# CogSP/CoEvoNet

Hardware: AMD Instinct MI355X
Metric: env-steps/sec (agent-steps of the whole job; generations/sec in gens_per_sec), Co-GA simple_adversary_v3 pop=200 HoF=5 (higher is better)
Workload: dtype f32

## Files before the change

### coevonet_amd/csrc/coevo_common.hip.h

```cpp
#pragma once
#include <hip/hip_runtime.h>
#include <stdint.h>

#include "../../include/coevo.h"

namespace coevo {

constexpr int H1 = COEVO_FC_H1;
constexpr int H2 = COEVO_FC_H2;
constexpr int NACT = COEVO_FC_NACT;
constexpr float LN_EPS = 1e-5f;

__host__ __device__ constexpr int64_t fc_off_b1(int D) { return (int64_t)D * H1; }
__host__ __device__ constexpr int64_t fc_off_w2(int D) { return fc_off_b1(D) + 3 * H1; }
__host__ __device__ constexpr int64_t fc_off_b2(int D) { return fc_off_w2(D) + (int64_t)H1 * H2; }
__host__ __device__ constexpr int64_t fc_off_w3(int D) { return fc_off_b2(D) + 3 * H2; }
__host__ __device__ constexpr int64_t fc_off_b3(int D) { return fc_off_w3(D) + NACT * H2; }
__host__ __device__ constexpr int64_t fc_params(int D) { return fc_off_b3(D) + NACT; }
__host__ __device__ constexpr int64_t fc_stride(int D) { return (fc_params(D) + 63) / 64 * 64; }

__host__ __device__ inline int64_t fc_slab_to_flat(int64_t s, int D)
{
    const int64_t o_b1 = fc_off_b1(D), o_w2 = fc_off_w2(D), o_b2 = fc_off_b2(D);
    if (s < o_b1) {
        int64_t k = s / H1, j = s % H1;
        return j * D + k;
    }
    if (s < o_w2) return s;
    if (s < o_b2) {
        int64_t t = s - o_w2;
        int64_t c = t & 3, l = (t >> 2) & 63, kq = (t >> 8) & 127, jb = t >> 15;
        return o_w2 + (jb * 64 + l) * H1 + kq * 4 + c;
    }
    return s;
}

template <int CTRL>
__device__ inline float dpp_move(float v)
{
    return __int_as_float(__builtin_amdgcn_mov_dpp(__float_as_int(v), CTRL, 0xf, 0xf, true));
}

__device__ inline float row16_tree_sum(float v)
{
    v = v + dpp_move<0xB1>(v);
    v = v + dpp_move<0x4E>(v);
    v = v + dpp_move<0x141>(v);
    v = v + dpp_move<0x140>(v);
    return v;
// ... 272 lines not shown
```

### coevonet_amd/csrc/fc_forward.hip

```cpp
#include <cstdlib>

#include "coevo_common.hip.h"

namespace coevo {

#ifndef COEVO_HEAVY16_U
#define COEVO_HEAVY16_U 4
#endif
#ifndef COEVO_LIGHT_U
#define COEVO_LIGHT_U 8
#endif

typedef float f32x4_t __attribute__((ext_vector_type(4)));
__device__ inline float4 load_stream16(const float4 *p)
{
#ifdef COEVO_NO_NT
    return *p;
#else
    const f32x4_t v = __builtin_nontemporal_load(reinterpret_cast<const f32x4_t *>(p));
    return make_float4(v[0], v[1], v[2], v[3]);
#endif
}

template <int R, int P>
// ... 1027 lines not shown
    fc_policy_mfma_body<MODE>(a, sm, a.tasks[blockIdx.x]);
}

struct FcMfma16Smem {
    union {
        float h1a[H1][16];
        float h2[16][260];
    };
    float xst[12][16];
    float w3s[NACT][260];
    float red[16][8];
    float logit[16][COEVO_LOGIT_STRIDE];
};
static_assert(sizeof(FcMfma16Smem) <= 40960, "four workgroups per CU");

template <int MODE>
__device__ __forceinline__ void fc_policy_mfma16_body(const FcArgs &a, FcMfma16Smem &sm, const coevo_fc_task &task)
{
    typedef float f32x4_acc __attribute__((ext_vector_type(4)));
    typedef unsigned u32x2_s __attribute__((ext_vector_type(2)));
    COEVO_STAMP(0);
    const int t = threadIdx.x, w = t >> 6, l = t & 63, lc = l & 15, lg = l >> 4;
    const int D = task.D, nrows = task.n_rows, row0 = task.row_begin;
    const float *net = a.slab + task.net_off;
    int st = 0;

    constexpr int KS = 3;
    float *par = &sm.h1a[0][0];
    {
        const int n_pieces = (D + 3) * (H1 / 4);
#pragma unroll
        for (int j = 0; j < 7; ++j)
            if (64 * w + 256 * j < n_pieces)
                __builtin_amdgcn_global_load_lds((const __attribute__((address_space(1))) void *)(net + 4 * (t + 256 * j)),
                                                 (__attribute__((address_space(3))) void *)(par + 4 * (64 * w + 256 * j)),
// ... 124 lines not shown
            if (row < nrows && bad_post_relu(y)) st |= COEVO_ST_BAD_FC1;
            const int k = 128 * w + 16 * T + lc;
            sm.h1a[k][row ^ ((k >> 2) & 3)] = relu_keep_nan(y);
        }
    }
    asm volatile("" : "+v"(st));
    __syncthreads();
    COEVO_STAMP(2);

    f32x4_acc c2[4];
    {
#pragma unroll
        for (int T = 0; T < 4; ++T)
#pragma unroll
            for (int i = 0; i < 4; ++i) c2[T][i] = p_b2[T];
        const float4 *wp = reinterpret_cast<const float4 *>(net + fc_off_w2(D)) + (size_t)w * 128 * 64 + l;
        constexpr int U = COEVO_HEAVY16_U;
        float4 bufA[U], bufB[U];
        auto issue = [&](float4 (&buf)[U], int kq) {
#pragma unroll
            for (int u = 0; u < U; ++u) buf[u] = wp[(size_t)(kq + u) * 64];
        };
        auto consume = [&](const float4 (&buf)[U], int kq) {
#pragma unroll
            for (int u = 0; u < U; ++u) {
                const int q = kq + u;
                const float av = sm.h1a[4 * q + lg][lc ^ (q & 3)];
                const u32x2_s s02 = __builtin_amdgcn_permlane32_swap(__float_as_uint(buf[u].x), __float_as_uint(buf[u].z), false, false);
                const u32x2_s s13 = __builtin_amdgcn_permlane32_swap(__float_as_uint(buf[u].y), __float_as_uint(buf[u].w), false, false);
                const u32x2_s y01 = __builtin_amdgcn_permlane16_swap(s02[0], s13[0], false, false);
                const u32x2_s y23 = __builtin_amdgcn_permlane16_swap(s02[1], s13[1], false, false);
                c2[0] = __builtin_amdgcn_mfma_f32_16x16x4f32(av, __uint_as_float(y01[0]), c2[0], 0, 0, 0);
                c2[1] = __builtin_amdgcn_mfma_f32_16x16x4f32(av, __uint_as_float(y01[1]), c2[1], 0, 0, 0);
                c2[2] = __builtin_amdgcn_mfma_f32_16x16x4f32(av, __uint_as_float(y23[0]), c2[2], 0, 0, 0);
                c2[3] = __builtin_amdgcn_mfma_f32_16x16x4f32(av, __uint_as_float(y23[1]), c2[3], 0, 0, 0);
            }
        };
        issue(bufA, 0);
        int kq = 0;
        for (; kq < 128 - 2 * U; kq += 2 * U) {
            issue(bufB, kq + U);
            __builtin_amdgcn_sched_barrier(0);
            consume(bufA, kq);
            issue(bufA, kq + 2 * U);
            __builtin_amdgcn_sched_barrier(0);
            consume(bufB, kq + U);
        }
        issue(bufB, kq + U);
        __builtin_amdgcn_sched_barrier(0);
        consume(bufA, kq);
// ... 82 lines not shown
}

template <int R, int MODE = MODE_FUSED>
__global__ __launch_bounds__(256, 4) void fc_cycle16_kernel(FcArgs a)
{
    __shared__ __attribute__((aligned(16))) union Cycle16Smem {
        FcMfma16Smem heavy;
#if COEVO_COMPACT
        FcSmemC<R> light;
#else
        FcSmem<R, 1> light;
#endif
    } sm;
    static_assert(sizeof(sm) <= 40960, "four workgroups per CU");
    stamp_begin(a.stamps);
    if ((int)blockIdx.x < a.n_heavy)
        fc_policy_mfma16_body<MODE>(a, sm.heavy, a.tasks[blockIdx.x]);
    else
#if COEVO_COMPACT
    {
        const int li = (int)blockIdx.x - a.n_heavy;
        if (MODE == MODE_FUSED && li < a.n_light && (a.light_tasks[li].reserved & COEVO_TASK_RESIDENT))
            fc_policy_body_c<R, MODE, FC2_MFMA, MODE == MODE_FUSED>(a, sm.light, a.light_tasks, li, a.n_light);
        else
            fc_policy_body_c<R, MODE>(a, sm.light, a.light_tasks, li, a.n_light);
    }
#else
        fc_policy_body<R, MODE, 1>(a, sm.light, a.light_tasks, (int)blockIdx.x - a.n_heavy, a.n_light);
#endif
    stamp_end(a.stamps);
}

template <int R, int MODE = MODE_FUSED>
// ... 684 lines not shown
```

### coevonet_amd/csrc/offspring.hip

```cpp
#include "coevo_common.hip.h"
#include "dqn_common.hip.h"
#include "philox.hip.h"

namespace coevo {

__device__ inline bool fc_slab_is_layernorm(int64_t s, int D)
{
    const int64_t g1 = fc_off_b1(D) + H1, g2 = fc_off_b2(D) + H2;
    return (s >= g1 && s < g1 + 2 * H1) || (s >= g2 && s < g2 + 2 * H2);
}

__device__ inline void slab_quad_normals(uint64_t seed, uint32_t slo, uint32_t shi, int64_t s0, int D, int64_t P,
                                         float z[4])
{
    int64_t p[4];
#pragma unroll
    for (int i = 0; i < 4; ++i) p[i] = (s0 + i < P) ? fc_slab_to_flat(s0 + i, D) : -1;
    float zz[4];
    int64_t have = -1;
#pragma unroll
    for (int i = 0; i < 4; ++i) {
        if (p[i] < 0) { z[i] = 0.0f; continue; }
        const int64_t q = p[i] >> 2;
        if (q != have) { philox_normal4(seed, slo, shi, (uint32_t)q, zz); have = q; }
// ... 130 lines not shown
    *reinterpret_cast<float4 *>(dst_slab + (int64_t)(dst_first + c) * stride + s0) = v;
}

struct GaPromoteArgs {
    coevo_ga_promote_role role[3];
    int E, hof;
    const float *sigma;
    const int32_t *gen_dev;
    uint64_t seed;
    uint32_t stream_hi_prev;
    int32_t *tick;
};
constexpr int PROMOTE_MAX_E = 8, PROMOTE_MAX_HOF = 16;

template <int I>
__device__ __forceinline__ void promote_hof_shift(float *hof, int64_t stride, int64_t s0, int n)
{
    if constexpr (I < PROMOTE_MAX_HOF) {
        const float4 v = *reinterpret_cast<const float4 *>(hof + (int64_t)(I < n ? I : n - 1) * stride + s0);
        promote_hof_shift<I + 1>(hof, stride, s0, n);
        *reinterpret_cast<float4 *>(hof + (int64_t)(I < n ? I - 1 : n - 1) * stride + s0) = v;
    }
}

template <int K>
__device__ __forceinline__ float4 promote_elites(const float *src, const int32_t *order, float *elite, bool store,
                                                 int64_t stride, int64_t s0, int E)
{
    if constexpr (K < PROMOTE_MAX_E) {
        const int kc = K < E ? K : E - 1;
        const float4 v = *reinterpret_cast<const float4 *>(src + (int64_t)(order ? order[kc] : kc) * stride + s0);
        promote_elites<K + 1>(src, order, elite, store, stride, s0, E);
        if (store) *reinterpret_cast<float4 *>(elite + (int64_t)kc * stride + s0) = v;
        return v;
    } else {
        return make_float4(0.f, 0.f, 0.f, 0.f);
// ... 23 lines not shown
        }
        *reinterpret_cast<float4 *>(elite + (int64_t)kc * stride + s0) = nv;
        return nv;
    } else {
        return make_float4(0.f, 0.f, 0.f, 0.f);
    }
}

__global__ __launch_bounds__(256) void ga_promote_kernel(GaPromoteArgs a)
{
    const unsigned y = blockIdx.y;
#define PROMOTE_SEL(f) (y == 0 ? a.role[0].f : (y == 1 ? a.role[1].f : a.role[2].f))
    float *pop = PROMOTE_SEL(pop), *hof = PROMOTE_SEL(hof), *elite = PROMOTE_SEL(elite);
    const int32_t *order = PROMOTE_SEL(order);
    const int D = PROMOTE_SEL(D), from_pop = PROMOTE_SEL(elites_from_pop), to_pop0 = PROMOTE_SEL(best_to_pop0);
#undef PROMOTE_SEL
    const int64_t stride = fc_stride(D);
    const int64_t s0 = ((int64_t)blockIdx.x * 256 + threadIdx.x) * 4;
    if (s0 >= stride) return;
    float4 e0;
    if (a.sigma && !from_pop) {
        uint32_t shi = a.stream_hi_prev + y;
        if (a.gen_dev) shi += 4u * (uint32_t)(*a.gen_dev - 1);
        e0 = promote_rebuild<0>(elite, order, stride, s0, a.E, D, a.sigma[y], a.seed, shi);
    } else {
        e0 = from_pop ? promote_elites<0>(pop, order, elite, true, stride, s0, a.E)
                      : *reinterpret_cast<const float4 *>(elite + s0);
    }
    promote_hof_shift<1>(hof, stride, s0, a.hof);
    *reinterpret_cast<float4 *>(hof + (int64_t)(a.hof - 1) * stride + s0) = e0;
    if (to_pop0) *reinterpret_cast<float4 *>(pop + s0) = e0;
    if (a.tick && blockIdx.x == 0 && blockIdx.y == 0 && threadIdx.x == 0) *a.tick += 1;
}

__global__ __launch_bounds__(256) void es_update_kernel(float *theta, const float *pert_slab, int D,
                                                         const float *fitness, int n, const float *sigma_dev, float lr)
{
    const int64_t stride = fc_stride(D), P = fc_params(D);
    const int64_t s0 = ((int64_t)blockIdx.x * 256 + threadIdx.x) * 4;
    if (s0 >= stride) return;
    const float sigma = *sigma_dev;
    const float scale = lr / ((float)n * sigma);
    const float4 tv = *reinterpret_cast<const float4 *>(theta + s0);
    const float th[4] = {tv.x, tv.y, tv.z, tv.w};
    float acc[4] = {0.0f, 0.0f, 0.0f, 0.0f};
// ... 242 lines not shown
                               int n, int D, void *stream)
{
    if (!src_slab || !src_idx || !dst_slab || !fc_dim_ok(D) || n < 0 || dst_first < 0 || n > 65535)
        return COEVO_ERR_ARG;
    if (n == 0) return COEVO_OK;
    const dim3 grid((unsigned)((fc_stride(D) / 4 + 255) / 256), (unsigned)n);
    hipLaunchKernelGGL(fc_gather_kernel, grid, dim3(256), 0, (hipStream_t)stream, src_slab, src_idx, dst_slab,
                       dst_first, fc_stride(D));
    COEVO_HIP_CHECK(hipGetLastError());
    return COEVO_OK;
}

static int ga_promote_launch(const coevo_ga_promote_role *roles, int n_roles, int E, int hof, const float *sigma,
                             uint64_t seed, uint32_t stream_hi_prev, const int32_t *gen_dev, int32_t *tick, void *stream);

extern "C" int coevo_ga_promote(const coevo_ga_promote_role *roles, int n_roles, int E, int hof, void *stream)
{
    return ga_promote_launch(roles, n_roles, E, hof, nullptr, 0, 0, nullptr, nullptr, stream);
}

extern "C" int coevo_ga_promote_tick(const coevo_ga_promote_role *roles, int n_roles, int E, int hof, int32_t *counter,
                                     void *stream)
{
    if (!counter) return COEVO_ERR_ARG;
    return ga_promote_launch(roles, n_roles, E, hof, nullptr, 0, 0, nullptr, counter, stream);
}

extern "C" int coevo_ga_promote_rebuild(const coevo_ga_promote_role *roles, int n_roles, int E, int hof, const float *sigma,
                                        uint64_t seed, uint32_t stream_hi_prev, const int32_t *gen_dev, void *stream)
{
// ... 1 lines not shown
    for (int r = 0; roles && r < n_roles && r < 3; ++r)
        if (!roles[r].elites_from_pop && !roles[r].order) return COEVO_ERR_ARG;
    return ga_promote_launch(roles, n_roles, E, hof, sigma, seed, stream_hi_prev, gen_dev, nullptr, stream);
}

static int ga_promote_launch(const coevo_ga_promote_role *roles, int n_roles, int E, int hof, const float *sigma,
                             uint64_t seed, uint32_t stream_hi_prev, const int32_t *gen_dev, int32_t *tick, void *stream)
{
    if (!roles || n_roles < 1 || n_roles > 3 || E < 1 || E > PROMOTE_MAX_E || hof < 1 || hof > PROMOTE_MAX_HOF)
        return COEVO_ERR_ARG;
    GaPromoteArgs a{};
    a.sigma = sigma; a.seed = seed; a.stream_hi_prev = stream_hi_prev; a.gen_dev = gen_dev; a.tick = tick;
    int64_t max_stride = 0;
    for (int r = 0; r < n_roles; ++r) {
        const coevo_ga_promote_role &R = roles[r];
        if (!R.pop || !R.hof || !R.elite || !fc_dim_ok(R.D) || (R.elites_from_pop && !R.order)) return COEVO_ERR_ARG;
        a.role[r] = R;
        if (fc_stride(R.D) > max_stride) max_stride = fc_stride(R.D);
    }
    a.E = E; a.hof = hof;
    const dim3 grid((unsigned)((max_stride / 4 + 255) / 256), (unsigned)n_roles);
    hipLaunchKernelGGL(ga_promote_kernel, grid, dim3(256), 0, (hipStream_t)stream, a);
    COEVO_HIP_CHECK(hipGetLastError());
    return COEVO_OK;
}

extern "C" int coevo_es_update(float *theta_slab_net, const float *pert_slab, int D, const float *fitness, int n,
                               const float *sigma_dev, float lr, void *stream)
{
    if (!theta_slab_net || !pert_slab || !fitness || !sigma_dev || !fc_dim_ok(D) || n <= 0) return COEVO_ERR_ARG;
    const dim3 grid((unsigned)((fc_stride(D) / 4 + 255) / 256));
// ... 141 lines not shown
```

### coevonet_amd/genetic_algorithm.py

```python
from __future__ import annotations

import os
import time

import numpy as np
import torch

from . import lib as L
from .fcnetwork import FCNetwork
from .game_logic import create_agent
from .mpe.simple_adversary import ENV_SEED
from .rollout import DeviceRollout, HostEnvRollout, RolloutPlan, effective_steps

ROLES = ("agent_0", "agent_1", "adversary_0")
ROLE_D = {"agent_0": 10, "agent_1": 10, "adversary_0": 8}
ROLE_SLOT = {"agent_0": 1, "agent_1": 2, "adversary_0": 0}
RET_SLOT = {"agent_0": 0, "agent_1": 1, "adversary_0": 2}
SIGMA_ATTR = {"agent_0": "mutation_power_agent_0", "agent_1": "mutation_power_agent_1",
              "adversary_0": "mutation_power_adversary"}
N_EVAL = 10


def evaluate_current_weights(agent_0, agent_1, adversary, env, args):
    from .game_logic import play_game
# ... 47 lines not shown
    return bounds, np.searchsorted(bounds[1:], np.arange(n_local), side="right").astype(np.int32)


RESIDENT_MB_DEFAULT = 224


def resident_budget_bytes():
    v = os.environ.get("COEVO_RESIDENT_MB", "").strip().lower()
    if v == "all":
        return float("inf")
    return (float(v) if v else RESIDENT_MB_DEFAULT) * 1e6


def resident_enabled(env, heavy_rows, n_local, pop):
    return env == "device" and heavy_rows == 16 and n_local >= pop


def resident_prefix(budget_bytes, fixed_bytes, individual_bytes, bounds):
    K = len(bounds) - 1
    sizes = np.diff(np.asarray(bounds, dtype=np.int64))
    left = budget_bytes - fixed_bytes
    if left <= 0 or K <= 0:
        return np.zeros(K, dtype=np.int64)
    if left == float("inf"):
        return sizes
    return np.minimum(sizes, int(left // (K * individual_bytes)))


DEFAULT_COHORTS = 1
DEVICE_LOOP_COHORTS = 2
# ... 15 lines not shown
        if self.world > 1 and pop % self.world:
            raise ValueError(f"population {pop} is not divisible by the number of ranks {self.world}")
        self.lo = self.rank * pop // self.world
        self.hi = (self.rank + 1) * pop // self.world
        self.n_local = self.hi - self.lo
        self.T_train = effective_steps(limit_train, max_cycles)
        self.T_eval = effective_steps(limit_eval, max_cycles)
        self.n_cycles = (max(self.T_train, self.T_eval) + 2) // 3
        self.first_ordinal = first_ordinal
        self.env_seed = env_seed
        self.stride = {r: L.fc_slab_stride(ROLE_D[r]) for r in ROLES}
        self.P = {r: L.fc_param_count(ROLE_D[r]) for r in ROLES}
        self.base, off = {}, 0
        for r in ROLES:
            self.base[r] = {}
            for region, count in (("pop", pop), ("hof", hof), ("elite", elites), ("stale", 1), ("hof_tmp", hof),
                                  ("elite_prev", elites)):
                self.base[r][region] = off
                off += count * self.stride[r]
        self.slab = torch.zeros(off, dtype=torch.float32, device=device)
        net_off, net_D, ids = [], [], {}

        def net(region, role, i):
            key = (region, role, i)
            if key not in ids:
                ids[key] = len(net_off)
                net_off.append(self.base[role][region] + i * self.stride[role])
                net_D.append(ROLE_D[role])
            return ids[key]

        games = []
        h = hof
# ... 11 lines not shown
        for _ in range(N_EVAL):
            games.append((net("hof", "adversary_0", h - 1), net("hof", "agent_0", h - 1), net("hof", "agent_1", h - 1)))
        heavy_rows = int(os.environ.get("COEVO_HEAVY_ROWS", "0"))
        if heavy_rows <= 0:
            cus = torch.cuda.get_device_properties(device).multi_processor_count if (env == "device" and str(device) != "cpu") else 0
            heavy_rows = small_shard_rows(self.n_local, hof, cus, pop) if (cus and cohorts <= 1) else 16
        host_k = int(os.environ.get("COEVO_HOST_COHORTS", "0")) or max(1, min(4, len(games) // 700))
        self.K = max(1, min(int(cohorts) if env == "device" else host_k, self.n_local))
        row_order = "class" if env == "device" else "cohort"
        self._set_cohort_bounds()
        game_cohort = None
        if self.K > 1:
            per_ind = np.repeat(cohort_partition(self.n_local, self.K)[1], self.hof)
            game_cohort = np.concatenate([per_ind, per_ind, per_ind, np.full(N_EVAL, self.K - 1)]).astype(np.int32)
        resident = resident_enabled(env, heavy_rows, self.n_local, pop)

        def resident_nets():
            if not resident:
                return ()
            ind_bytes = sum(4 * self.stride[r] for r in ROLES)
            n = resident_prefix(resident_budget_bytes(), (hof + elites + 1) * ind_bytes, ind_bytes, self.cohort_bounds)
            return [ids[("pop", r, self.lo + i)] for r in ROLES for k in range(self.K)
                    for i in range(int(self.cohort_bounds[k]), int(self.cohort_bounds[k]) + int(n[k]))]

        try:
            self.plan = RolloutPlan(np.array(games), net_off, net_D, device=device, heavy_rows=heavy_rows,
                                    n_cohorts=self.K, game_cohort=game_cohort, row_order=row_order,
                                    resident_nets=resident_nets())
        except ValueError:
            self.K = 1
            self._set_cohort_bounds()
            self.plan = RolloutPlan(np.array(games), net_off, net_D, device=device, heavy_rows=heavy_rows,
                                    row_order=row_order, resident_nets=resident_nets())
        if env == "device":
            self.ro = DeviceRollout(self.plan, self.slab, env_seed=env_seed, timing_pairs=timing_pairs)
        else:
            self.ro = HostEnvRollout(self.plan, self.slab, env_seed=env_seed)
        f32 = dict(dtype=torch.float32, device=device)
        self.dist_all = torch.zeros(3, pop, **f32)
        self.dist = {r: self.dist_all[i] for i, r in enumerate(ROLES)}
        self.div = {r: torch.zeros(1, **f32) for r in ROLES}
        self.fitness = {r: torch.zeros(pop, **f32) for r in ROLES}
        self.order = {r: torch.zeros(pop, dtype=torch.int32, device=device) for r in ROLES}
        self.sigma = {r: torch.zeros(1, **f32) for r in ROLES}
        self.sigma_prev = {r: torch.zeros(1, **f32) for r in ROLES}
        self.last_reward = torch.zeros(3, pop, 3, dtype=torch.float64, device=device)
        self.pack_local = torch.zeros(3, self.n_local, 4, dtype=torch.float64, device=device)
        self.pack_all = torch.zeros(self.world, 3, self.n_local, 4, dtype=torch.float64, device=device)
        self.parent_idx = torch.tensor([c % elites for c in range(max(pop - 1, 1))], dtype=torch.int32, device=device)
        self.hof_shift_idx = torch.arange(1, max(hof, 2), dtype=torch.int32, device=device)
        self.iota = torch.arange(max(hof, elites, 2), dtype=torch.int32, device=device)
        self.generation = 0
        self.steps_per_generation = 3 * pop * hof * self.T_train + N_EVAL * self.T_eval

    def _ptr(self, role, region, i=0):
        return self.slab.data_ptr() + 4 * (self.base[role][region] + i * self.stride[role])

    def upload(self, role, region, first, flat_np):
        flat = torch.from_numpy(np.ascontiguousarray(flat_np, dtype=np.float32)).to(self.device)
        L.call("coevo_fc_pack", L._p(flat), self._ptr(role, region, first), flat.shape[0], ROLE_D[role])
        if region in ("pop", "stale"):
            self._dist_current = False
        return flat

    def download(self, role, region, first, n):
        if region == "pop":
            self.flush_breeding()
        out = torch.zeros(n, self.P[role], dtype=torch.float32, device=self.device)
        L.call("coevo_fc_unpack", self._ptr(role, region, first), L._p(out), n, ROLE_D[role])
        return out.cpu().numpy()

    def load_initial(self, pop_flat, hof_flat):
        keep = []
        for r in ROLES:
            keep.append(self.upload(r, "pop", 0, pop_flat[r]))
# ... 120 lines not shown
            L.call("coevo_fc_gather", self._ptr(r, "elite"), L._p(self.iota), self._ptr(r, "pop"), 0, 1, D)
            c_lo, c_hi = (max(self.lo, 1) - 1, self.hi - 1) if sharded else (0, self.pop - 1)
            if c_hi > c_lo:
                L.call("coevo_fc_perturb", self._ptr(r, "elite"), self.parent_idx.data_ptr() + 4 * c_lo,
                       self._ptr(r, "pop"), 1 + c_lo, c_hi - c_lo, D, L._p(self.sigma[r]), self.philox_seed, c_lo,
                       gen * 4 + ri, 0)

    def _hof_push(self, r):
        D = ROLE_D[r]
        if self.hof > 1:
            L.call("coevo_fc_gather", self._ptr(r, "hof"), L._p(self.hof_shift_idx), self._ptr(r, "hof_tmp"), 0,
                   self.hof - 1, D)
            L.call("coevo_fc_gather", self._ptr(r, "hof_tmp"), L._p(self.iota), self._ptr(r, "hof"), 0,
                   self.hof - 1, D)
        L.call("coevo_fc_gather", self._ptr(r, "elite"), L._p(self.iota), self._ptr(r, "hof"), self.hof - 1, 1, D)

    def breed_host_reference(self, env, args, sigmas):
        keep = []
        self._dist_current = False
        for r in ROLES:
            D = ROLE_D[r]
            L.call("coevo_fc_gather", self._ptr(r, "pop"), L._p(self.order[r]), self._ptr(r, "elite"), 0, self.E, D)
            self._hof_push(r)
            L.call("coevo_fc_gather", self._ptr(r, "elite"), L._p(self.iota), self._ptr(r, "pop"), 0, 1, D)
        elite_flat = {r: self.download(r, "elite", 0, self.E) for r in ROLES}
        for r in ROLES:
            children = np.empty((self.pop - 1, self.P[r]), dtype=np.float32)
            for i in range(self.pop - 1):
                child = FCNetwork(ROLE_D[r], 5, "float32")
                child.set_flat(elite_flat[r][i % self.E])
# ... 54 lines not shown
        roles = (L.GaSelectRole * 3)()
        for ri, r in enumerate(ROLES):
            roles[ri] = L.GaSelectRole(None if gathered is not None else L._p(self.dist[r]),
                                       None if gathered is not None else rewards_ptr_of(ri), L._p(self.div[r]),
                                       L._p(self.fitness[r]), L._p(self.order[r]), L._p(self.best_dist[r]),
                                       0 if gathered is not None else game_first_of(ri), RET_SLOT[r])
        ad = self._adapt_args(with_prev)
        L.call("coevo_ga_select_adapt", roles, 3, self.pop, games_per_individual, self.hof,
               L._p(gathered) if gathered is not None else None, self.n_local if gathered is not None else 0, L.C.byref(ad))

    def _promote_roles(self, elites_from_pop, best_to_pop0, tick=False):
        roles = (L.GaPromoteRole * 3)()
        for ri, r in enumerate(ROLES):
            roles[ri] = L.GaPromoteRole(self._ptr(r, "pop"), self._ptr(r, "hof"), self._ptr(r, "elite"),
                                        L._p(self.order[r]), ROLE_D[r], 1 if elites_from_pop else 0,
                                        1 if best_to_pop0 else 0, 0)
        if tick:
            L.call("coevo_ga_promote_tick", roles, 3, self.E, self.hof, L._p(self.gen_dev))
            return
        L.call("coevo_ga_promote", roles, 3, self.E, self.hof)

    def enqueue_generation(self):
        self._enqueue_resets()
        self.ro.enqueue(self.n_cycles)
        self._enqueue_selection_and_breeding()

    def _enqueue_resets(self):
        assert self.world == 1 and self.env_mode == "device"
        ro, M = self.ro, 3 * self.pop * self.hof
        per_gen, per_phase = M + N_EVAL, self.pop * self.hof
        g = L._p(self.gen_dev)
# ... 191 lines not shown
                    self._sharded_tail_post(gen, breed=breed, gen_from_device=True, packed=packed)
                graphs[key] = gr
            graphs[key].replay()
            return
        self._sharded_tail_post(gen, breed, gen_from_device=False, packed=packed)

    def _sharded_tail_post(self, gen, breed, gen_from_device, packed=False):
        ro = self.ro
        g = L._p(self.gen_dev)
        mn, mx, adaptive = self.loop_args
        if packed:
            self._select_adapt_roles(None, None, 1, gathered=self.pack_all, with_prev=True)
            pr = (L.GaPromoteRole * 3)()
            for ri, r in enumerate(ROLES):
                pr[ri] = L.GaPromoteRole(self._ptr(r, "pop"), self._ptr(r, "hof"), self._ptr(r, "elite"), L._p(self.order[r]),
                                         ROLE_D[r], 1 if gen == 0 else 0, 1 if self.lo == 0 else 0, 0)
            if gen == 0:
                L.call("coevo_ga_promote", pr, 3, self.E, self.hof)
            else:
                L.call("coevo_ga_promote_rebuild", pr, 3, self.E, self.hof, L._p(self.sigma32_prev), self.philox_seed,
                       0 if gen_from_device else (gen - 1) * 4, g if gen_from_device else None)
            if breed:
                self._breed_cohort(0, gen, gen_dev=g if gen_from_device else None, tick=True)
            else:
                L.call("coevo_counter_add", g, 1)
            return
        if self.fused_tail:
            self._select_roles(lambda ri: self.last_reward[ri].data_ptr(), lambda ri: 0, 1)
        else:
            for ph, r in enumerate(ROLES):
                L.call("coevo_sharing_score", L._p(self.dist[r]), self.pop, L._p(self.div[r]))
# ... 292 lines not shown
```

### coevonet_amd/lib.py

```python
from __future__ import annotations

import ctypes as C
import os

import numpy as np
import torch

HERE = os.path.dirname(os.path.abspath(__file__))
LIB_PATH = os.environ.get("COEVO_LIB") or os.path.join(HERE, "libcoevo.so")

OBS_STRIDE = 12
LOGIT_STRIDE = 8
FC_MAX_ROWS = 32
MPE_STATE_DOUBLES = 24
STAMP_SLOTS = 32
ST_NAMES = {1: "input contains inf or NaN", 2: "output contains inf or NaN after fc1",
            4: "output contains inf or NaN after fc2", 8: "output contains inf or NaN",
            16: "no action selected (current_best_position = -1)",
            32: "persistent rollout: a workgroup timed out waiting for the other rows of its games (COEVO_ST_SYNC_TIMEOUT)",
            64: "fp16 forward: a task with a bad width, row count or unaligned net offset was skipped (COEVO_ST_BAD_TASK)"}

DQN_LOGIT_STRIDE = 32
DQN_FC1_TILED = 0x100
DQN_MAX_ROWS = 16
DQN_TASK_DTYPE = np.dtype([("net_off", "<i8"), ("row_begin", "<i4"), ("n_rows", "<i4")])

TASK_DTYPE = np.dtype([("net_off", "<i8"), ("row_begin", "<i4"), ("n_rows", "<i4"), ("D", "<i4"),
                       ("reserved", "<i4")])
TASK_RESIDENT = 1


class PCG64State(C.Structure):
    _fields_ = [("state_hi", C.c_uint64), ("state_lo", C.c_uint64), ("inc_hi", C.c_uint64), ("inc_lo", C.c_uint64)]

    @classmethod
    def from_seed(cls, seed):
        st = np.random.PCG64(seed).state["state"]
        m = (1 << 64) - 1
        return cls(st["state"] >> 64, st["state"] & m, st["inc"] >> 64, st["inc"] & m)


class PerturbJob(C.Structure):
    _fields_ = [("parent_slab", C.c_void_p), ("parent_idx", C.c_void_p), ("child_slab", C.c_void_p),
                ("sigma_dev", C.c_void_p), ("dist_ref", C.c_void_p), ("dist_partial", C.c_void_p),
# ... 214 lines not shown
    "coevo_fc_rebuild_elites": (C.c_int, [C.c_void_p, C.c_void_p, C.c_void_p, C.c_int, C.c_int, C.c_void_p, C.c_uint64,
                                          C.c_uint32, C.c_void_p, C.c_void_p]),
    "coevo_fc_perturb_gen": (C.c_int, [C.c_void_p, C.c_void_p, C.c_void_p, C.c_int, C.c_int, C.c_int, C.c_void_p,
                                       C.c_uint64, C.c_uint32, C.c_uint32, C.c_int, C.c_void_p, C.c_void_p]),
    "coevo_fc_perturb_blocks": (C.c_int64, [C.c_int]),
    "coevo_fc_perturb_dist": (C.c_int, [C.c_void_p, C.c_void_p, C.c_void_p, C.c_int, C.c_int, C.c_int, C.c_void_p,
                                        C.c_uint64, C.c_uint32, C.c_uint32, C.c_int, C.c_void_p, C.c_void_p, C.c_void_p,
                                        C.c_void_p]),
    "coevo_fc_distance_finalize": (C.c_int, [C.c_void_p, C.c_int, C.c_int, C.c_void_p, C.c_int, C.c_void_p,
                                             C.c_void_p]),
    "coevo_gather_f32": (C.c_int, [C.c_void_p, C.c_void_p, C.c_void_p, C.c_int, C.c_void_p]),
    "coevo_ga_adapt_sigma": (C.c_int, [C.c_void_p, C.c_int, C.c_void_p, C.c_void_p, C.c_void_p, C.c_int, C.c_void_p,
                                       C.c_void_p, C.c_double, C.c_double, C.c_int, C.c_void_p]),
    "coevo_counter_add": (C.c_int, [C.c_void_p, C.c_int, C.c_void_p]),
    "coevo_fc_gather": (C.c_int, [C.c_void_p, C.c_void_p, C.c_void_p, C.c_int, C.c_int, C.c_int, C.c_void_p]),
    "coevo_es_update": (C.c_int, [C.c_void_p, C.c_void_p, C.c_int, C.c_void_p, C.c_int, C.c_void_p, C.c_float,
                                  C.c_void_p]),
    "coevo_fc_diversity": (C.c_int, [C.c_void_p, C.c_void_p, C.c_int, C.c_int, C.c_void_p, C.c_void_p, C.c_void_p]),
    "coevo_fc_distance": (C.c_int, [C.c_void_p, C.c_void_p, C.c_int, C.c_int, C.c_void_p, C.c_void_p]),
    "coevo_sharing_score": (C.c_int, [C.c_void_p, C.c_int, C.c_void_p, C.c_void_p]),
    "coevo_ga_fitness": (C.c_int, [C.c_void_p, C.c_int, C.c_int, C.c_int, C.c_int, C.c_int, C.c_void_p, C.c_void_p,
                                   C.c_void_p]),
    "coevo_rank_desc": (C.c_int, [C.c_void_p, C.c_int, C.c_void_p, C.c_void_p]),
}


def exported_symbols():
    return sorted(_SIGS)


# ... 85 lines not shown
```

### coevonet_amd/rollout.py

```python
from __future__ import annotations

import ctypes as _ct

import os

import numpy as np
import torch

from . import lib as L
from .mpe import simple_adversary as sa

LIGHT_ROWS = 8
HEAVY_ROWS = 32


class RolloutPlan:

    def __init__(self, game_nets, net_off, net_D, device="cuda", heavy_rows=HEAVY_ROWS, n_cohorts=1,
                 game_cohort=None, split_rows=None, row_order="class", resident_nets=()):
        game_nets = np.asarray(game_nets, dtype=np.int64)
        self.n_games = int(game_nets.shape[0])
        by_net = {}
        for g in range(self.n_games):
            for slot in range(3):
                by_net.setdefault(int(game_nets[g, slot]), []).append((g, slot))
        for net, rows in by_net.items():
            d = int(net_D[net])
            for g, slot in rows:
                assert d == (8 if slot == 0 else 10), "net width does not match the env slot it plays"
        if game_cohort is not None:
            cohort = np.asarray(game_cohort, dtype=np.int32)
            assert cohort.shape == (self.n_games,) and cohort.min() >= 0
            for net, rows in by_net.items():
                if len(rows) <= LIGHT_ROWS and len({int(cohort[g]) for g, _ in rows}) != 1:
# ... 15 lines not shown
                light[int(cohort[rows[0][0]])].append((net, rows))
            else:
                for k in range(self.n_cohorts):
                    mine = [(g, slot) for g, slot in rows if cohort[g] == k]
                    for i in range(0, len(mine), heavy_rows):
                        heavy[k].append((net, mine[i:i + heavy_rows]))
        heavy = [self._xcd_order(h) for h in heavy]
        self.heavy_begin_np = np.cumsum([0] + [len(h) for h in heavy]).astype(np.int32)
        self.light_begin_np = np.cumsum([0] + [len(x) for x in light]).astype(np.int32)
        assert row_order in ("class", "cohort")
        row_game, row_slot = [], []
        tasks = {"heavy": [[] for _ in range(self.n_cohorts)], "light": [[] for _ in range(self.n_cohorts)]}
        cohort_rows = np.zeros(self.n_cohorts + 1, dtype=np.int64)

        resident_nets = frozenset(int(n) for n in resident_nets)

        def number(name, k):
            for net, rows in (heavy if name == "heavy" else light)[k]:
                flags = L.TASK_RESIDENT if (name == "light" and net in resident_nets) else 0
                tasks[name][k].append((int(net_off[net]), len(row_game), len(rows), int(net_D[net]), flags))
                for g, slot in rows:
                    row_game.append(g)
                    row_slot.append(slot)

        if row_order == "class":
            for name in ("heavy", "light"):
                for k in range(self.n_cohorts):
                    number(name, k)
            self.cohort_row_begin_np = None
        else:
            for k in range(self.n_cohorts):
                number("heavy", k)
                number("light", k)
                cohort_rows[k + 1] = len(row_game)
# ... 462 lines not shown
```

### include/coevo.h

```cpp
#ifndef COEVO_H
#define COEVO_H

#include <stddef.h>
#include <stdint.h>

#ifdef __cplusplus
extern "C" {
#endif

#define COEVO_VERSION 103

#define COEVO_OK 0
#define COEVO_ERR_ARG (-1)
#define COEVO_ERR_HIP (-2)
#define COEVO_ERR_UNSUPPORTED (-3)

#define COEVO_ST_BAD_INPUT 1
#define COEVO_ST_BAD_FC1 2
#define COEVO_ST_BAD_FC2 4
#define COEVO_ST_BAD_OUT 8
#define COEVO_ST_NO_ACTION 16
#define COEVO_ST_SYNC_TIMEOUT 32
#define COEVO_ST_BAD_TASK 64

// ... 13 lines not shown
const char *coevo_build_flags(void);

int64_t coevo_fc_param_count(int D);
int64_t coevo_fc_slab_stride(int D);
int coevo_fc_pack(const float *flat, float *slab, int n, int D, void *stream);
int coevo_fc_unpack(const float *slab, float *flat, int n, int D, void *stream);

typedef struct {
    int64_t net_off;
    int32_t row_begin;
    int32_t n_rows;
    int32_t D;
    int32_t reserved;
} coevo_fc_task;
#define COEVO_TASK_RESIDENT 1

int coevo_fc_forward_argmax(const float *slab, const coevo_fc_task *tasks, int n_tasks, int max_rows_per_task,
                            const float *obs, int32_t *actions, float *logits, int32_t *status, void *stream);
int coevo_fc_forward_merged(const float *slab, const coevo_fc_task *heavy_tasks, int n_heavy, int heavy_max_rows,
                            const coevo_fc_task *light_tasks, int n_light, int light_max_rows, const float *obs,
                            int32_t *actions, float *logits, int32_t *status, void *stream);

int64_t coevo_fc16_slab_stride(int D);
int coevo_fc16_pack(const float *flat, void *slab, int n, int D, void *stream);
int coevo_fc16_unpack(const void *slab, float *flat, int n, int D, void *stream);
int coevo_fc16_forward_argmax(const void *slab, const coevo_fc_task *tasks, int n_tasks, int max_rows_per_task,
                              const float *obs, int32_t *actions, float *logits, int32_t *status, void *stream);

#define COEVO_MPE_STATE_DOUBLES 24
typedef struct {
// ... 200 lines not shown
int coevo_ga_select(const coevo_ga_select_role *roles, int n_roles, int pop, int games_per_individual, int hof,
                    void *stream);
int coevo_ga_select_gathered(const coevo_ga_select_role *roles, int n_roles, int pop, int hof, const double *gathered,
                             int n_local, void *stream);
typedef struct coevo_ga_adapt_args {
    const double *rewards; const int32_t *gen_dev; double *hist; double *sig_hist; double *sigma64; float *sigma32;
    float *sigma32_prev; double sig_min, sig_max; int32_t eval_first_game, cap, adaptive, reserved;
} coevo_ga_adapt_args;
int coevo_ga_select_adapt(const coevo_ga_select_role *roles, int n_roles, int pop, int games_per_individual, int hof,
                          const double *gathered, int n_local, const coevo_ga_adapt_args *adapt, void *stream);
typedef struct coevo_ga_promote_role {
    float *pop, *hof, *elite;
    const int32_t *order;
    int32_t D, elites_from_pop, best_to_pop0, reserved;
} coevo_ga_promote_role;
int coevo_ga_promote(const coevo_ga_promote_role *roles, int n_roles, int E, int hof, void *stream);
int coevo_ga_promote_tick(const coevo_ga_promote_role *roles, int n_roles, int E, int hof, int32_t *counter, void *stream);
int coevo_ga_promote_rebuild(const coevo_ga_promote_role *roles, int n_roles, int E, int hof, const float *sigma,
                             uint64_t seed, uint32_t stream_hi_prev, const int32_t *gen_dev, void *stream);
int coevo_fc_gather(const float *src_slab, const int32_t *src_idx, float *dst_slab, int dst_first, int n, int D,
                    void *stream);

int coevo_es_update(float *theta_slab_net, const float *pert_slab, int D, const float *fitness, int n,
                    const float *sigma_dev, float lr, void *stream);

int coevo_es_partial(const float *theta_net, const float *pert_slab_local, int ind_first, int D,
                     const float *fitness_all, int n_total, int chunks_total, int chunk_first, int n_chunks,
                     float *partial, void *stream);
int coevo_es_apply(float *theta_net, const float *partials, int chunks_total, int chunks_per_block,
                   int64_t block_stride_floats, int D, int n_total, const float *sigma_dev, float lr, void *stream);
// ... 103 lines not shown
```

Baseline: 147.8 million.

## Keep pre-swizzled W2 twin copies of hall-of-fame nets to skip lane permutes

Adds a twin region holding the W2 weights of each hall-of-fame network already permuted into MFMA operand order. The copy is kept up to date on upload, on rebuild and during promote shifts. Heavy forward tasks flagged as tiled read the twin and skip four permlane swaps per MFMA group in the inner W2 loop. This costs extra slab memory and extra writes during promotion, and it helps only the heavy tasks that evaluate HoF nets.

```diff
diff --git a/coevonet_amd/csrc/coevo_common.hip.h b/coevonet_amd/csrc/coevo_common.hip.h
--- a/coevonet_amd/csrc/coevo_common.hip.h
+++ b/coevonet_amd/csrc/coevo_common.hip.h
@@ -33,6 +33,16 @@
         return o_w2 + (jb * 64 + l) * H1 + kq * 4 + c;
     }
     return s;
+}
+
+__device__ __forceinline__ float4 w2_twin_piece(float4 v)
+{
+    typedef unsigned u32x2_t __attribute__((ext_vector_type(2)));
+    const u32x2_t s02 = __builtin_amdgcn_permlane32_swap(__float_as_uint(v.x), __float_as_uint(v.z), false, false);
+    const u32x2_t s13 = __builtin_amdgcn_permlane32_swap(__float_as_uint(v.y), __float_as_uint(v.w), false, false);
+    const u32x2_t y01 = __builtin_amdgcn_permlane16_swap(s02[0], s13[0], false, false);
+    const u32x2_t y23 = __builtin_amdgcn_permlane16_swap(s02[1], s13[1], false, false);
+    return make_float4(__uint_as_float(y01[0]), __uint_as_float(y01[1]), __uint_as_float(y23[0]), __uint_as_float(y23[1]));
 }
 
 template <int CTRL>
diff --git a/coevonet_amd/csrc/fc_forward.hip b/coevonet_amd/csrc/fc_forward.hip
--- a/coevonet_amd/csrc/fc_forward.hip
+++ b/coevonet_amd/csrc/fc_forward.hip
@@ -1065,11 +1065,10 @@
 };
 static_assert(sizeof(FcMfma16Smem) <= 40960, "four workgroups per CU");
 
-template <int MODE>
+template <int MODE, bool TILED = false>
 __device__ __forceinline__ void fc_policy_mfma16_body(const FcArgs &a, FcMfma16Smem &sm, const coevo_fc_task &task)
 {
     typedef float f32x4_acc __attribute__((ext_vector_type(4)));
-    typedef unsigned u32x2_s __attribute__((ext_vector_type(2)));
     COEVO_STAMP(0);
     const int t = threadIdx.x, w = t >> 6, l = t & 63, lc = l & 15, lg = l >> 4;
     const int D = task.D, nrows = task.n_rows, row0 = task.row_begin;
@@ -1224,7 +1223,8 @@
         for (int T = 0; T < 4; ++T)
 #pragma unroll
             for (int i = 0; i < 4; ++i) c2[T][i] = p_b2[T];
-        const float4 *wp = reinterpret_cast<const float4 *>(net + fc_off_w2(D)) + (size_t)w * 128 * 64 + l;
+        const float *w2 = TILED ? net + (int64_t)(task.reserved >> COEVO_TASK_TWIN_SHIFT) * fc_stride(D) : net;
+        const float4 *wp = reinterpret_cast<const float4 *>(w2 + fc_off_w2(D)) + (size_t)w * 128 * 64 + l;
         constexpr int U = COEVO_HEAVY16_U;
         float4 bufA[U], bufB[U];
         auto issue = [&](float4 (&buf)[U], int kq) {
@@ -1236,14 +1236,11 @@
             for (int u = 0; u < U; ++u) {
                 const int q = kq + u;
                 const float av = sm.h1a[4 * q + lg][lc ^ (q & 3)];
-                const u32x2_s s02 = __builtin_amdgcn_permlane32_swap(__float_as_uint(buf[u].x), __float_as_uint(buf[u].z), false, false);
-                const u32x2_s s13 = __builtin_amdgcn_permlane32_swap(__float_as_uint(buf[u].y), __float_as_uint(buf[u].w), false, false);
-                const u32x2_s y01 = __builtin_amdgcn_permlane16_swap(s02[0], s13[0], false, false);
-                const u32x2_s y23 = __builtin_amdgcn_permlane16_swap(s02[1], s13[1], false, false);
-                c2[0] = __builtin_amdgcn_mfma_f32_16x16x4f32(av, __uint_as_float(y01[0]), c2[0], 0, 0, 0);
-                c2[1] = __builtin_amdgcn_mfma_f32_16x16x4f32(av, __uint_as_float(y01[1]), c2[1], 0, 0, 0);
-                c2[2] = __builtin_amdgcn_mfma_f32_16x16x4f32(av, __uint_as_float(y23[0]), c2[2], 0, 0, 0);
-                c2[3] = __builtin_amdgcn_mfma_f32_16x16x4f32(av, __uint_as_float(y23[1]), c2[3], 0, 0, 0);
+                const float4 b = TILED ? buf[u] : w2_twin_piece(buf[u]);
+                c2[0] = __builtin_amdgcn_mfma_f32_16x16x4f32(av, b.x, c2[0], 0, 0, 0);
+                c2[1] = __builtin_amdgcn_mfma_f32_16x16x4f32(av, b.y, c2[1], 0, 0, 0);
+                c2[2] = __builtin_amdgcn_mfma_f32_16x16x4f32(av, b.z, c2[2], 0, 0, 0);
+                c2[3] = __builtin_amdgcn_mfma_f32_16x16x4f32(av, b.w, c2[3], 0, 0, 0);
             }
         };
         issue(bufA, 0);
@@ -1356,9 +1353,12 @@
     } sm;
     static_assert(sizeof(sm) <= 40960, "four workgroups per CU");
     stamp_begin(a.stamps);
-    if ((int)blockIdx.x < a.n_heavy)
-        fc_policy_mfma16_body<MODE>(a, sm.heavy, a.tasks[blockIdx.x]);
-    else
+    if ((int)blockIdx.x < a.n_heavy) {
+        if (MODE == MODE_FUSED && (a.tasks[blockIdx.x].reserved & COEVO_TASK_W2_TILED))
+            fc_policy_mfma16_body<MODE, MODE == MODE_FUSED>(a, sm.heavy, a.tasks[blockIdx.x]);
+        else
+            fc_policy_mfma16_body<MODE>(a, sm.heavy, a.tasks[blockIdx.x]);
+    } else
 #if COEVO_COMPACT
     {
         const int li = (int)blockIdx.x - a.n_heavy;
diff --git a/coevonet_amd/csrc/offspring.hip b/coevonet_amd/csrc/offspring.hip
--- a/coevonet_amd/csrc/offspring.hip
+++ b/coevonet_amd/csrc/offspring.hip
@@ -168,12 +168,14 @@
 constexpr int PROMOTE_MAX_E = 8, PROMOTE_MAX_HOF = 16;
 
 template <int I>
-__device__ __forceinline__ void promote_hof_shift(float *hof, int64_t stride, int64_t s0, int n)
+__device__ __forceinline__ void promote_hof_shift(float *hof, int64_t stride, int64_t s0, int n, int twin)
 {
     if constexpr (I < PROMOTE_MAX_HOF) {
         const float4 v = *reinterpret_cast<const float4 *>(hof + (int64_t)(I < n ? I : n - 1) * stride + s0);
-        promote_hof_shift<I + 1>(hof, stride, s0, n);
-        *reinterpret_cast<float4 *>(hof + (int64_t)(I < n ? I - 1 : n - 1) * stride + s0) = v;
+        promote_hof_shift<I + 1>(hof, stride, s0, n, twin);
+        const int64_t slot = I < n ? I - 1 : n - 1;
+        *reinterpret_cast<float4 *>(hof + slot * stride + s0) = v;
+        if (twin > 0) *reinterpret_cast<float4 *>(hof + (slot + twin) * stride + s0) = w2_twin_piece(v);
     }
 }
 
@@ -227,6 +229,7 @@
     float *pop = PROMOTE_SEL(pop), *hof = PROMOTE_SEL(hof), *elite = PROMOTE_SEL(elite);
     const int32_t *order = PROMOTE_SEL(order);
     const int D = PROMOTE_SEL(D), from_pop = PROMOTE_SEL(elites_from_pop), to_pop0 = PROMOTE_SEL(best_to_pop0);
+    const int twin = PROMOTE_SEL(reserved);
 #undef PROMOTE_SEL
     const int64_t stride = fc_stride(D);
     const int64_t s0 = ((int64_t)blockIdx.x * 256 + threadIdx.x) * 4;
@@ -240,8 +243,11 @@
         e0 = from_pop ? promote_elites<0>(pop, order, elite, true, stride, s0, a.E)
                       : *reinterpret_cast<const float4 *>(elite + s0);
     }
-    promote_hof_shift<1>(hof, stride, s0, a.hof);
+    const int64_t s_wave = s0 - 4 * (int64_t)(threadIdx.x & 63);
+    const int tw = (twin > 0 && s_wave >= fc_off_w2(D) && s_wave < fc_off_b2(D)) ? twin : 0;
+    promote_hof_shift<1>(hof, stride, s0, a.hof, tw);
     *reinterpret_cast<float4 *>(hof + (int64_t)(a.hof - 1) * stride + s0) = e0;
+    if (tw > 0) *reinterpret_cast<float4 *>(hof + (int64_t)(a.hof - 1 + tw) * stride + s0) = w2_twin_piece(e0);
     if (to_pop0) *reinterpret_cast<float4 *>(pop + s0) = e0;
     if (a.tick && blockIdx.x == 0 && blockIdx.y == 0 && threadIdx.x == 0) *a.tick += 1;
 }
@@ -514,6 +520,24 @@
 static int ga_promote_launch(const coevo_ga_promote_role *roles, int n_roles, int E, int hof, const float *sigma,
                              uint64_t seed, uint32_t stream_hi_prev, const int32_t *gen_dev, int32_t *tick, void *stream);
 
+__global__ __launch_bounds__(256) void fc_w2_tile_kernel(const float *src, float *dst, int64_t stride, int64_t w2)
+{
+    const int64_t s0 = w2 + ((int64_t)blockIdx.x * 256 + threadIdx.x) * 4;
+    const int64_t net = (int64_t)blockIdx.y * stride;
+    const float4 v = *reinterpret_cast<const float4 *>(src + net + s0);
+    *reinterpret_cast<float4 *>(dst + net + s0) = w2_twin_piece(v);
+}
+
+extern "C" int coevo_fc_w2_tile(const float *src, float *dst, int n, int D, void *stream)
+{
+    if (!src || !dst || n < 0 || !fc_dim_ok(D)) return COEVO_ERR_ARG;
+    if (n == 0) return COEVO_OK;
+    const dim3 grid((unsigned)(H1 * H2 / 1024), (unsigned)n);
+    hipLaunchKernelGGL(fc_w2_tile_kernel, grid, dim3(256), 0, (hipStream_t)stream, src, dst, fc_stride(D), fc_off_w2(D));
+    COEVO_HIP_CHECK(hipGetLastError());
+    return COEVO_OK;
+}
+
 extern "C" int coevo_ga_promote(const coevo_ga_promote_role *roles, int n_roles, int E, int hof, void *stream)
 {
     return ga_promote_launch(roles, n_roles, E, hof, nullptr, 0, 0, nullptr, nullptr, stream);
@@ -545,7 +569,8 @@
     int64_t max_stride = 0;
     for (int r = 0; r < n_roles; ++r) {
         const coevo_ga_promote_role &R = roles[r];
-        if (!R.pop || !R.hof || !R.elite || !fc_dim_ok(R.D) || (R.elites_from_pop && !R.order)) return COEVO_ERR_ARG;
+        if (!R.pop || !R.hof || !R.elite || !fc_dim_ok(R.D) || (R.elites_from_pop && !R.order) || R.reserved < 0)
+            return COEVO_ERR_ARG;
         a.role[r] = R;
         if (fc_stride(R.D) > max_stride) max_stride = fc_stride(R.D);
     }
diff --git a/coevonet_amd/genetic_algorithm.py b/coevonet_amd/genetic_algorithm.py
--- a/coevonet_amd/genetic_algorithm.py
+++ b/coevonet_amd/genetic_algorithm.py
@@ -85,6 +85,10 @@
 
 def resident_enabled(env, heavy_rows, n_local, pop):
     return env == "device" and heavy_rows == 16 and n_local >= pop
+
+
+def heavy_tiled_enabled(env, heavy_rows, n_local, pop):
+    return os.environ.get("COEVO_HEAVY_TILED", "1").strip() != "0" and resident_enabled(env, heavy_rows, n_local, pop)
 
 
 def resident_prefix(budget_bytes, fixed_bytes, individual_bytes, bounds):
@@ -130,8 +134,8 @@
         self.base, off = {}, 0
         for r in ROLES:
             self.base[r] = {}
-            for region, count in (("pop", pop), ("hof", hof), ("elite", elites), ("stale", 1), ("hof_tmp", hof),
-                                  ("elite_prev", elites)):
+            for region, count in (("pop", pop), ("hof", hof), ("hof_w2t", hof), ("elite", elites), ("stale", 1),
+                                  ("hof_tmp", hof), ("elite_prev", elites)):
                 self.base[r][region] = off
                 off += count * self.stride[r]
         self.slab = torch.zeros(off, dtype=torch.float32, device=device)
@@ -173,6 +177,10 @@
             per_ind = np.repeat(cohort_partition(self.n_local, self.K)[1], self.hof)
             game_cohort = np.concatenate([per_ind, per_ind, per_ind, np.full(N_EVAL, self.K - 1)]).astype(np.int32)
         resident = resident_enabled(env, heavy_rows, self.n_local, pop)
+        self.w2_tiled = heavy_tiled_enabled(env, heavy_rows, self.n_local, pop)
+
+        def tiled_nets():
+            return {i: hof for (region, _, _), i in ids.items() if region == "hof"} if self.w2_tiled else None
 
         def resident_nets():
             if not resident:
@@ -185,12 +193,12 @@
         try:
             self.plan = RolloutPlan(np.array(games), net_off, net_D, device=device, heavy_rows=heavy_rows,
                                     n_cohorts=self.K, game_cohort=game_cohort, row_order=row_order,
-                                    resident_nets=resident_nets())
+                                    resident_nets=resident_nets(), tiled_nets=tiled_nets())
         except ValueError:
             self.K = 1
             self._set_cohort_bounds()
             self.plan = RolloutPlan(np.array(games), net_off, net_D, device=device, heavy_rows=heavy_rows,
-                                    row_order=row_order, resident_nets=resident_nets())
+                                    row_order=row_order, resident_nets=resident_nets(), tiled_nets=tiled_nets())
         if env == "device":
             self.ro = DeviceRollout(self.plan, self.slab, env_seed=env_seed, timing_pairs=timing_pairs)
         else:
@@ -218,6 +226,8 @@
     def upload(self, role, region, first, flat_np):
         flat = torch.from_numpy(np.ascontiguousarray(flat_np, dtype=np.float32)).to(self.device)
         L.call("coevo_fc_pack", L._p(flat), self._ptr(role, region, first), flat.shape[0], ROLE_D[role])
+        if region == "hof":
+            self._tile_hof(role)
         if region in ("pop", "stale"):
             self._dist_current = False
         return flat
@@ -368,6 +378,11 @@
             L.call("coevo_fc_gather", self._ptr(r, "hof_tmp"), L._p(self.iota), self._ptr(r, "hof"), 0,
                    self.hof - 1, D)
         L.call("coevo_fc_gather", self._ptr(r, "elite"), L._p(self.iota), self._ptr(r, "hof"), self.hof - 1, 1, D)
+        self._tile_hof(r)
+
+    def _tile_hof(self, r):
+        if self.w2_tiled:
+            L.call("coevo_fc_w2_tile", self._ptr(r, "hof"), self._ptr(r, "hof_w2t"), self.hof, ROLE_D[r])
 
     def breed_host_reference(self, env, args, sigmas):
         keep = []
@@ -452,7 +467,7 @@
         for ri, r in enumerate(ROLES):
             roles[ri] = L.GaPromoteRole(self._ptr(r, "pop"), self._ptr(r, "hof"), self._ptr(r, "elite"),
                                         L._p(self.order[r]), ROLE_D[r], 1 if elites_from_pop else 0,
-                                        1 if best_to_pop0 else 0, 0)
+                                        1 if best_to_pop0 else 0, self.hof if self.w2_tiled else 0)
         if tick:
             L.call("coevo_ga_promote_tick", roles, 3, self.E, self.hof, L._p(self.gen_dev))
             return
@@ -674,7 +689,8 @@
             pr = (L.GaPromoteRole * 3)()
             for ri, r in enumerate(ROLES):
                 pr[ri] = L.GaPromoteRole(self._ptr(r, "pop"), self._ptr(r, "hof"), self._ptr(r, "elite"), L._p(self.order[r]),
-                                         ROLE_D[r], 1 if gen == 0 else 0, 1 if self.lo == 0 else 0, 0)
+                                         ROLE_D[r], 1 if gen == 0 else 0, 1 if self.lo == 0 else 0,
+                                         self.hof if self.w2_tiled else 0)
             if gen == 0:
                 L.call("coevo_ga_promote", pr, 3, self.E, self.hof)
             else:
diff --git a/coevonet_amd/lib.py b/coevonet_amd/lib.py
--- a/coevonet_amd/lib.py
+++ b/coevonet_amd/lib.py
@@ -28,6 +28,8 @@
 TASK_DTYPE = np.dtype([("net_off", "<i8"), ("row_begin", "<i4"), ("n_rows", "<i4"), ("D", "<i4"),
                        ("reserved", "<i4")])
 TASK_RESIDENT = 1
+TASK_W2_TILED = 2
+TASK_TWIN_SHIFT = 8
 
 
 class PCG64State(C.Structure):
@@ -272,6 +274,7 @@
                                        C.c_void_p, C.c_double, C.c_double, C.c_int, C.c_void_p]),
     "coevo_counter_add": (C.c_int, [C.c_void_p, C.c_int, C.c_void_p]),
     "coevo_fc_gather": (C.c_int, [C.c_void_p, C.c_void_p, C.c_void_p, C.c_int, C.c_int, C.c_int, C.c_void_p]),
+    "coevo_fc_w2_tile": (C.c_int, [C.c_void_p, C.c_void_p, C.c_int, C.c_int, C.c_void_p]),
     "coevo_es_update": (C.c_int, [C.c_void_p, C.c_void_p, C.c_int, C.c_void_p, C.c_int, C.c_void_p, C.c_float,
                                   C.c_void_p]),
     "coevo_fc_diversity": (C.c_int, [C.c_void_p, C.c_void_p, C.c_int, C.c_int, C.c_void_p, C.c_void_p, C.c_void_p]),
diff --git a/coevonet_amd/rollout.py b/coevonet_amd/rollout.py
--- a/coevonet_amd/rollout.py
+++ b/coevonet_amd/rollout.py
@@ -17,7 +17,7 @@
 class RolloutPlan:
 
     def __init__(self, game_nets, net_off, net_D, device="cuda", heavy_rows=HEAVY_ROWS, n_cohorts=1,
-                 game_cohort=None, split_rows=None, row_order="class", resident_nets=()):
+                 game_cohort=None, split_rows=None, row_order="class", resident_nets=(), tiled_nets=None):
         game_nets = np.asarray(game_nets, dtype=np.int64)
         self.n_games = int(game_nets.shape[0])
         by_net = {}
@@ -63,10 +63,13 @@
         cohort_rows = np.zeros(self.n_cohorts + 1, dtype=np.int64)
 
         resident_nets = frozenset(int(n) for n in resident_nets)
+        tiled_nets = {int(n): int(k) for n, k in (tiled_nets or {}).items()}
 
         def number(name, k):
             for net, rows in (heavy if name == "heavy" else light)[k]:
                 flags = L.TASK_RESIDENT if (name == "light" and net in resident_nets) else 0
+                if name == "heavy" and net in tiled_nets:
+                    flags |= L.TASK_W2_TILED | (tiled_nets[net] << L.TASK_TWIN_SHIFT)
                 tasks[name][k].append((int(net_off[net]), len(row_game), len(rows), int(net_D[net]), flags))
                 for g, slot in rows:
                     row_game.append(g)
diff --git a/include/coevo.h b/include/coevo.h
--- a/include/coevo.h
+++ b/include/coevo.h
@@ -51,6 +51,8 @@
     int32_t reserved;
 } coevo_fc_task;
 #define COEVO_TASK_RESIDENT 1
+#define COEVO_TASK_W2_TILED 2
+#define COEVO_TASK_TWIN_SHIFT 8
 
 int coevo_fc_forward_argmax(const float *slab, const coevo_fc_task *tasks, int n_tasks, int max_rows_per_task,
                             const float *obs, int32_t *actions, float *logits, int32_t *status, void *stream);
@@ -281,6 +283,7 @@
     const int32_t *order;
     int32_t D, elites_from_pop, best_to_pop0, reserved;
 } coevo_ga_promote_role;
+int coevo_fc_w2_tile(const float *src, float *dst, int n, int D, void *stream);
 int coevo_ga_promote(const coevo_ga_promote_role *roles, int n_roles, int E, int hof, void *stream);
 int coevo_ga_promote_tick(const coevo_ga_promote_role *roles, int n_roles, int E, int hof, int32_t *counter, void *stream);
 int coevo_ga_promote_rebuild(const coevo_ga_promote_role *roles, int n_roles, int E, int hof, const float *sigma,
```

New measurement: 149.6 million, median of 6. +1.2%, better.
